# 14chanwa/remotesensingProject

Measured on AMD Instinct MI355X. Metric: Mpixel*disparity-hypotheses/s, higher is better.
Workload: dtype f32

## Files before the change

### remotesensingproject_amd/csrc/k2_reg.hpp

```cpp
#pragma once

#include "k2_scan.hpp"

namespace rslf {

#ifndef RSLF_REG_GB104
#define RSLF_REG_GB104 8
#endif
constexpr int gather_batch(int c) { return c == 1 ? 8 : 4; }
constexpr int kPadSlack = 16;

template <int SPAD, int C, bool BORDER, bool UNIFORM_D, bool PK, int GB = 0, class BestT = Best<C>, bool LANE_D = false>
__device__ __forceinline__ void scan_reg_body(const ScanArgs& a, int v, int u, int d0, int d1, BestT& best,
                                              float* __restrict__ otab, int dlane = 0, int dstep = 1)
{
    static_assert(!LANE_D || !UNIFORM_D, "hypotheses in the lanes: every lane has its own view offsets");
    constexpr int kGatherBatch = GB > 0 ? GB : (C == 1 && !PK && SPAD == 104 && RSLF_REG_GB104 == 13) ? 13 : gather_batch(C);
    static_assert(SPAD % kGatherBatch == 0 && (!PK || kGatherBatch % 2 == 0), "whole batches, whole pairs");
    static_assert(SPAD % 8 == 0, "slot counts are multiples of 8");
    const VolView& vol = a.vol;
    const float* epi = vol.row(v, 0);
    const float uf = (float)u;
    const int Um1 = vol.U - 1;
    const unsigned Um1_bits = __float_as_uint((float)Um1);
    const int S = vol.S;
    const int lane = threadIdx.x & 63;
    const long long o = (long long)v * vol.U + u;
    const float dmin = a.dmin_vu ? a.dmin_vu[o] : a.dmin;
    const float dmax = a.dmax_vu ? a.dmax_vu[o] : a.dmax;
    const float range = dmax - dmin;
    const float denom = (float)(a.dim_d - 1);
    const float kq = (C == 1) ? a.k.k1 : a.k.inv_h2;
    const float slope = a.k.slope;
    const int stride_s = (int)vol.stride_s;
    float centre[C];
#pragma unroll
    for (int c = 0; c < C; c++)
        centre[c] = epi[(long long)a.s_hat * vol.stride_s + u * C + c];

#pragma unroll 1
    for (int dk = d0; dk < d1; dk += (LANE_D ? dstep : 1)) {
        const int d = LANE_D ? min(dk + dlane, d1 - 1) : dk;
        const float Dd = hypothesis(dmin, range, denom, d);
        float R[PK ? 1 : C][PK ? 1 : SPAD];
        f2 R2[PK ? C : 1][PK ? SPAD / 2 : 1];
        int card = BORDER ? 0 : S;
        float Ss0 = (float)a.s_hat;
        asm volatile("" : "+v"(Ss0));
        int rowoff = 0;
        asm volatile("" : "+s"(rowoff));
        if (UNIFORM_D) {
#pragma unroll
            for (int s0 = 0; s0 < SPAD; s0 += 64) {
                const int s = s0 + lane;
                float off = (float)(a.s_hat - s) * Dd;
                off = off * slope;
                if (SPAD % 64 == 0 || s < SPAD)
                    otab[s] = off;
            }
            __builtin_amdgcn_wave_barrier();
        }
#pragma unroll
        for (int g = 0; g < SPAD / kGatherBatch; g++) {
            float tt[kGatherBatch], e0[C][kGatherBatch], e1[C][kGatherBatch];
            bool ok[kGatherBatch];
#pragma unroll
            for (int j = 0; j < kGatherBatch; j++) {
                const int s = g * kGatherBatch + j;
                tt[j] = 0.0f;
                ok[j] = false;
#pragma unroll
                for (int c = 0; c < C; c++) {
                    e0[c][j] = kSentinel;
                    e1[c][j] = 0.0f;
                }
                if (s < SPAD - kPadSlack || s < S) {
                    float x;
                    if (UNIFORM_D) {
                        x = otab[s];
                    } else {
                        x = (Ss0 - (float)s) * Dd;
                        x = x * slope;
                    }
                    x = x + uf;
                    tt[j] = lerp_weight(x);
                    int i0 = floor_to_int(x);
                    ok[j] = true;
                    if (BORDER) {
                        ok[j] = __float_as_uint(x) <= Um1_bits;
                        i0 = ok[j] ? i0 : 0;
                    }
                    const unsigned byteoff = (unsigned)(i0 * C + rowoff) << 2;
                    const float* p = (const float*)((const char*)epi + byteoff);
#pragma unroll
                    for (int c = 0; c < C; c++) {
                        e0[c][j] = p[c];
                        e1[c][j] = p[C + c];
                    }
                }
                rowoff += stride_s;
            }
#pragma unroll
            for (int j = 0; j < kGatherBatch; j++) {
                const int s = g * kGatherBatch + j;
                const float omt = 1.0f - tt[j];
#pragma unroll
                for (int c = 0; c < C; c++) {
                    const float m0 = omt * e0[c][j];
                    const float m1 = tt[j] * e1[c][j];
                    const float r = m0 + m1;
                    float val;
                    if (BORDER)
                        val = ok[j] ? r : kSentinel;
                    else
                        val = (s < SPAD - kPadSlack || s < S) ? r : kSentinel;
                    if constexpr (PK) {
                        if (s & 1)
                            R2[c][s >> 1].y = val;
                        else
                            R2[c][s >> 1].x = val;
                    } else {
                        R[c][s] = val;
                    }
                }
                if (BORDER)
                    card += ok[j] ? 1 : 0;
            }
            {
                const int b = g * kGatherBatch;
#pragma unroll
                for (int c = 0; c < C; c++) {
                    if constexpr (PK) {
                        asm volatile("" : "+v"(R2[c][b / 2]), "+v"(R2[c][b / 2 + 1]));
                        if (kGatherBatch == 8)
                            asm volatile("" : "+v"(R2[c][b / 2 + 2]), "+v"(R2[c][b / 2 + 3]));
                        static_assert(!PK || kGatherBatch == 4 || kGatherBatch == 8, "pair pinning is written for 4 and 8");
                    } else if (kGatherBatch != 4 && kGatherBatch != 8) {
#pragma unroll
                        for (int j = 0; j < kGatherBatch; j++)
                            asm volatile("" : "+v"(R[c][b + j]));
                    } else {
                        asm volatile("" : "+v"(R[c][b + 0]), "+v"(R[c][b + 1]), "+v"(R[c][b + 2]), "+v"(R[c][b + 3]));
                        if (kGatherBatch == 8)
                            asm volatile("" : "+v"(R[c][b + kGatherBatch - 4]), "+v"(R[c][b + kGatherBatch - 3]),
                                              "+v"(R[c][b + kGatherBatch - 2]), "+v"(R[c][b + kGatherBatch - 1]));
                    }
                }
                if (BORDER)
                    asm volatile("" : "+s"(rowoff), "+v"(Ss0), "+v"(card));
                else
                    asm volatile("" : "+s"(rowoff), "+v"(Ss0));
            }
        }

        float rbar[C];
#pragma unroll
        for (int c = 0; c < C; c++)
            rbar[c] = centre[c];
        float B = 0.0f;
#pragma unroll 1
        for (int it = 0; it < a.k.n_iter; it++) {
            float A[C];
#pragma unroll
            for (int c = 0; c < C; c++)
                A[c] = 0.0f;
            B = 0.0f;
            if constexpr (PK) {
                f2 rb2[C];
                const f2 kq2 = {kq, kq};
#pragma unroll
                for (int c = 0; c < C; c++)
                    rb2[c] = f2{rbar[c], rbar[c]};
                constexpr int kBlk = (C == 1) ? 8 : 4;
#pragma unroll
                for (int s0 = 0; s0 < SPAD; s0 += kBlk) {
                    if (!(s0 < SPAD - kPadSlack || s0 < S))
                        continue;
                    if constexpr (C == 1) {
                        f2 P[4], K[4];
                        const f2 r4[4] = {R2[0][s0 / 2], R2[0][s0 / 2 + 1], R2[0][s0 / 2 + 2], R2[0][s0 / 2 + 3]};
                        mean_shift_pk_octet(r4, rb2[0], kq2, P, K);
#pragma unroll
                        for (int j = 0; j < 4; j++) {
                            A[0] = A[0] + P[j].x;
                            B = B + K[j].x;
                            A[0] = A[0] + P[j].y;
                            B = B + K[j].y;
                        }
                    } else {
                        f2 Pa[3], Pb[3], Ka, Kb;
                        const f2 ra[3] = {R2[0][s0 / 2], R2[1][s0 / 2], R2[C - 1][s0 / 2]};
                        const f2 rb[3] = {R2[0][s0 / 2 + 1], R2[1][s0 / 2 + 1], R2[C - 1][s0 / 2 + 1]};
                        const f2 m[3] = {rb2[0], rb2[C > 1 ? 1 : 0], rb2[C - 1]};
                        mean_shift_pk_rgb_quad(ra, rb, m, kq2, Pa, Pb, Ka, Kb);
#pragma unroll
                        for (int c = 0; c < C; c++)
                            A[c] = A[c] + Pa[c].x;
                        B = B + Ka.x;
#pragma unroll
                        for (int c = 0; c < C; c++)
                            A[c] = A[c] + Pa[c].y;
                        B = B + Ka.y;
#pragma unroll
                        for (int c = 0; c < C; c++)
                            A[c] = A[c] + Pb[c].x;
                        B = B + Kb.x;
#pragma unroll
                        for (int c = 0; c < C; c++)
                            A[c] = A[c] + Pb[c].y;
                        B = B + Kb.y;
                    }
                }
            } else if (C == 1) {
#pragma unroll
                for (int s0 = 0; s0 < SPAD; s0 += 4) {
                    if (s0 + 4 <= SPAD - kPadSlack || s0 + 4 <= S) {
                        mean_shift_group4(R[0][s0], R[0][s0 + 1], R[0][s0 + 2], R[0][s0 + 3], rbar[0], kq, A[0], B);
                    } else {
#pragma unroll
                        for (int j = 0; j < 3; j++)
                            if (s0 + j < S)
                                mean_shift_group1(R[0][s0 + j], rbar[0], kq, A[0], B);
                    }
                }
            } else {
#pragma unroll
                for (int s = 0; s < SPAD; s++) {
                    if (!(s < SPAD - kPadSlack || s < S))
                        continue;
                    float q[C];
#pragma unroll
                    for (int c = 0; c < C; c++) {
                        const float delta = R[c][s] - rbar[c];
                        const float tq = kq * delta;
                        q[c] = tq * delta;
                    }
                    float qs = q[0];
                    if (C == 3) {
                        qs = q[0] + q[C - 1];
                        qs = qs + q[C > 1 ? 1 : 0];
                    }
                    const float K = kernel_weight(qs);
#pragma unroll
                    for (int c = 0; c < C; c++) {
                        const float pr = R[c][s] * K;
                        A[c] = A[c] + pr;
                    }
                    B = B + K;
                }
            }
#pragma unroll
            for (int c = 0; c < C; c++) {
                const float qd = (B != 0.0f) ? (A[c] / B) : 0.0f;
                rbar[c] = (qd > 0.0f) ? qd : 0.0f;
            }
        }
        const float cardf = (float)card;
        float sc = (card != 0) ? (B / cardf) : 0.0f;
        sc = (sc > 0.0f) ? sc : 0.0f;
        if (!LANE_D || dk + dlane < d1)
            best.offer(sc, d, Dd, rbar);
    }
}

constexpr int scan_reg_waves(int spad, int c)
{
    const int regs = ((c * spad + (c == 1 ? 64 : 96) + 7) / 8) * 8;
    const int w = 512 / regs;
    if (c == 1 && spad > 104 && spad <= 144) return 3;
    if (c == 1 && spad >= 80 && spad <= 88) return 4;
    if (c == 3 && spad >= 32 && spad <= 40) return 3;
    if (c == 1 && (spad == 48 || spad == 40)) return 5;
    if (c == 3 && spad == 24) return 4;
    if (c == 1 && spad == 16) return 7;
    return w > 8 ? 8 : (w < 1 ? 1 : w);
}

#ifndef RSLF_REG_BEST_LDS
#define RSLF_REG_BEST_LDS 1
#endif
constexpr bool scan_reg_best_in_lds(int spad, int c)
{
    if (!RSLF_REG_BEST_LDS)
        return false;
    if (c == 1)
        return spad == 16 || spad == 40 || spad == 48 || (spad >= 80 && spad <= 88) || (spad >= 104 && spad <= 144);
    return spad == 24 || spad == 40;
}

constexpr bool scan_reg_packed_math(int spad, int c) { return scan_reg_waves(spad, c) == 1; }

template <int SPAD, int C, class BestT>
__device__ __forceinline__ void scan_reg_rows(const ScanArgs& a, int v, int u, int d0, int d1, BestT& best, float* otab)
{
    constexpr bool PK = scan_reg_packed_math(SPAD, C);
    if (a.dmin_vu) {
        scan_reg_body<SPAD, C, true, false, PK, 0, BestT>(a, v, u, d0, d1, best, otab);
        return;
    }
    const float max_ds = (float)max(a.s_hat, a.vol.S - 1 - a.s_hat);
    const float range = a.dmax - a.dmin, denom = (float)(a.dim_d - 1);
    const float uf = (float)u, Um1 = (float)(a.vol.U - 1);
    auto interior = [&](int d) -> bool {
        const float reach = max_ds * fabsf(hypothesis(a.dmin, range, denom, d)) * fabsf(a.k.slope) + 2.0f;
        return __all((uf - reach >= 0.0f) && (uf + reach <= Um1));
    };
    int d = d0;
    while (d < d1) {
        const bool in = interior(d);
        int e = d + 1;
        while (e < d1 && interior(e) == in)
            e++;
        if (in)
            scan_reg_body<SPAD, C, false, true, PK, 0, BestT>(a, v, u, d, e, best, otab);
        else
            scan_reg_body<SPAD, C, true, true, PK, 0, BestT>(a, v, u, d, e, best, otab);
        d = e;
    }
}

template <int SPAD, int C>
__global__ __launch_bounds__(64 * kScanWaves) __attribute__((amdgpu_waves_per_eu(scan_reg_waves(SPAD, C), scan_reg_waves(SPAD, C))))
void k2_scan_reg(ScanArgs a)
{
    __shared__ float s_otab[kScanWaves][SPAD];
    float* otab = s_otab[__builtin_amdgcn_readfirstlane(threadIdx.x >> 6)];
    constexpr bool kEpiDyn = false;
    float* const epi_lds = nullptr;
    const int epi_stride = 0;
    if constexpr (scan_reg_best_in_lds(SPAD, C)) {
        __shared__ float s_best[kScanWaves][BestLds<C>::kFloats];
        BestLds<C> running(s_best[__builtin_amdgcn_readfirstlane(threadIdx.x >> 6)]);
        RSLF_SCAN_ROW_TILE((running.init(), scan_reg_rows<SPAD, C>(a, v, u, d0, d1, running, otab), running.load(best)))
    } else {
        RSLF_SCAN_ROW_TILE((scan_reg_rows<SPAD, C>(a, v, u, d0, d1, best, otab)))
    }
}

#ifndef RSLF_PACKED_LONG_GB
#define RSLF_PACKED_LONG_GB 4
#endif
constexpr bool packed_long_unit(int spad, int c) { return c == 1 && spad >= 80 && spad <= 128 && spad % RSLF_PACKED_LONG_GB == 0; }
constexpr int packed_waves(int spad, int c) { return packed_long_unit(spad, c) ? 2 : scan_reg_waves(spad + 24, c); }
constexpr int packed_gather_batch(int spad, int c) { return packed_long_unit(spad, c) ? spad / RSLF_PACKED_LONG_GB : 0; }

template <int SPAD, int C>
__global__ __launch_bounds__(64 * kScanWaves) __attribute__((amdgpu_waves_per_eu(packed_waves(SPAD, C), packed_waves(SPAD, C))))
void k2_scan_reg_packed(ScanArgs a)
{
    constexpr bool kEpiDyn = false;
    float* const epi_lds = nullptr;
    const int epi_stride = 0;
    RSLF_SCAN_PACKED_LOOP((scan_reg_body<SPAD, C, true, false, packed_waves(SPAD, C) == 1, packed_gather_batch(SPAD, C)>(a, v, u, d0, d1, best, nullptr)))
}

#ifndef RSLF_PX_ROWLIKE
#define RSLF_PX_ROWLIKE 1
#endif
constexpr int px_kernel_waves(int spad, int c) { return RSLF_PX_ROWLIKE ? scan_reg_waves(spad, c) : packed_waves(spad, c); }
template <int SPAD, int C>
__global__ __launch_bounds__(64 * kScanWaves) __attribute__((amdgpu_waves_per_eu(px_kernel_waves(SPAD, C), px_kernel_waves(SPAD, C))))
void k2_scan_reg_px(ScanArgs a)
{
    __shared__ double s_sum[kScanWaves];
    __shared__ float s_rec[kScanWaves][kPxRecFloats];
    const int n = *a.packed_n;
    const int lane = threadIdx.x & 63;
    const int wave = __builtin_amdgcn_readfirstlane(threadIdx.x >> 6);
    const int wpp = a.px_waves, ppw = kScanWaves / wpp;
    const int items = (n + ppw - 1) / ppw;
    const int sub = wave % wpp;
    const int dlane = sub * 64 + lane, dstep = 64 * wpp;
    for (int item = blockIdx.x; item < items; item += gridDim.x) {
        const int e = item * ppw + wave / wpp;
        const bool listed = e < n;
        const unsigned o = (unsigned)__builtin_amdgcn_readfirstlane(a.list[listed ? e : n - 1]);
        const int v = (int)(o / (unsigned)a.vol.U);
        const int u = (int)(o - (unsigned)v * (unsigned)a.vol.U);
        const bool have = listed && scan_px_owns(a, v);
        Best<C> best;
        best.init();
        const float dlo = a.dmin_vu ? a.dmin_vu[o] : a.dmin, dhi = a.dmax_vu ? a.dmax_vu[o] : a.dmax;
        const float reach = (float)max(a.s_hat, a.vol.S - 1 - a.s_hat) * fmaxf(fabsf(dlo), fabsf(dhi)) * fabsf(a.k.slope) + 2.0f;
        const bool interior = (float)u - reach >= 0.0f && (float)u + reach <= (float)(a.vol.U - 1);
        constexpr int kGB = RSLF_PX_ROWLIKE ? 0 : packed_gather_batch(SPAD, C);
        if (!have) {
        } else if (interior)
            scan_reg_body<SPAD, C, false, false, false, kGB, Best<C>, true>(a, v, u, 0, a.dim_d, best, nullptr, dlane, dstep);
        else
            scan_reg_body<SPAD, C, true, false, false, kGB, Best<C>, true>(a, v, u, 0, a.dim_d, best, nullptr, dlane, dstep);
        scan_px_finish<C>(a, o, have, best, wave, lane, wpp, s_rec, s_sum);
    }
}

}
```

### remotesensingproject_amd/csrc/k2_scan.hpp

```cpp
#pragma once

#include <type_traits>

#include "rslf_device.hpp"

namespace rslf {

constexpr int kScanWaves = 4;
#ifndef RSLF_XCD_ROW_INTERLEAVE
#define RSLF_XCD_ROW_INTERLEAVE 1
#endif

struct ScanArgs {
    VolView vol;
    const int* list;
    const int* count;
    const float* dmin_vu;
    const float* dmax_vu;
    float dmin, dmax;
    int dim_d, s_hat;
    ScanConsts k;
    float* Ce;
    uint8_t* Ce_mask;
    float* Cd;
// ... 85 lines not shown
            blk[0] = sc;
            reinterpret_cast<int*>(blk)[64] = dd;
            blk[128] = Dd;
#pragma unroll
            for (int c = 0; c < C; c++)
                blk[(3 + c) * 64] = rb[c];
        }
    }
    __device__ __forceinline__ void load(Best<C>& b) const
    {
        b.score = blk[0];
        b.d = reinterpret_cast<const int*>(blk)[64];
        b.D = blk[128];
#pragma unroll
        for (int c = 0; c < C; c++)
            b.rbar[c] = blk[(3 + c) * 64];
        b.sum = *sum_ptr();
    }
};

__device__ __forceinline__ bool scan_tile_span(const ScanArgs& a, int lb, int& v, int& e0, int& width, int& n)
{
    if (lb >= a.logical_blocks)
        return false;
    const int tile = lb / a.groups;
    const int vr = tile / a.tiles_per_row;
    const int j = tile - vr * a.tiles_per_row;
    v = vr + a.v0;
    n = a.count[v];
    if (j * a.tile_w >= n || n < a.row_min)
        return false;
    width = a.tile_w;
    if (a.tile_w == 63) {
        const int T = max(1, (n + 61) / 63);
        if (j >= T)
            return false;
        if (j == T - 1)
            width = n - 63 * j;
    }
    e0 = j * a.tile_w;
    return true;
}
__device__ __forceinline__ bool scan_tile(const ScanArgs& a, int lb, int& v, int& u, bool& active, int lane = threadIdx.x & 63)
{
    int e0, width, n;
    if (!scan_tile_span(a, lb, v, e0, width, n))
        return false;
    const int e = e0 + lane;
    active = lane < width && e < n;
    const int idx = active ? e : min(e0 + width, n) - 1;
    if (a.rowbase)
        u = a.list[a.rowbase[v] + idx] - v * a.vol.U;
    else
        u = a.list[(long long)v * a.vol.U + idx];
    return true;
}

__device__ __forceinline__ void scan_tile_packed(const ScanArgs& a, int item, int n, int& v, int& u, bool& active)
{
    const int lane = threadIdx.x & 63;
    const int e = (item / a.groups) * 64 + lane;
    active = e < n;
    const unsigned o = (unsigned)a.list[active ? e : n - 1];
    v = (int)(o / (unsigned)a.vol.U);
    u = (int)(o - (unsigned)v * (unsigned)a.vol.U);
}

__device__ __forceinline__ void scan_chunk(const ScanArgs& a, int group, int& d0, int& d1)
{
    const int wave = __builtin_amdgcn_readfirstlane(threadIdx.x >> 6);
    const int slices = kScanWaves * a.groups;
    const int chunk = (a.dim_d + slices - 1) / slices;
    d0 = min((group * kScanWaves + wave) * chunk, a.dim_d);
    d1 = min(d0 + chunk, a.dim_d);
}

__device__ __forceinline__ float hypothesis(float dmin, float range, float denom, int d)
{
    const float num = (float)d * range;
    const float quo = num / denom;
    return dmin + quo;
}

template <int C>
__device__ __forceinline__ void write_pixel(const ScanArgs& a, long long o, float best, int best_d, float best_D,
                                            const float (&best_rbar)[C], double sum)
{
    if ((double)best > (double)a.k.raw_thr) {
        a.depth[o] = best_D;
        const double mean = sum / (double)a.dim_d;
        a.Cd[o] = (float)((double)a.Ce[o] * fabs((double)best - mean));
#pragma unroll
        for (int c = 0; c < C; c++)
            a.rbar[o * C + c] = best_rbar[c];
        if (a.idx)
            a.idx[o] = best_d;
        if (a.score)
            a.score[o] = best;
    } else {
        a.Ce[o] = 0.0f;
        a.Ce_mask[o] = 0;
    }
}

constexpr int kPxRecFloats = 3 + 3;
__device__ __forceinline__ bool scan_px_owns(const ScanArgs& a, int v)
{
    return a.row_min == 0 || a.count[v] < a.row_min;
}

template <int C>
__device__ __forceinline__ void scan_px_finish(const ScanArgs& a, unsigned o, bool have, const Best<C>& best, int wave, int lane, int wpp,
                                               float (*rec)[kPxRecFloats], double* wsum)
{
    const int sub = wave % wpp;
    float bs = best.score;
    int bd = bs < 0.0f ? 0x7fffffff : best.d;
    double sum = best.sum;
#pragma unroll
    for (int m = 32; m >= 1; m >>= 1) {
        const float os = __shfl_xor(bs, m);
        const int od = __shfl_xor(bd, m);
        const bool take = os > bs || (os == bs && od < bd);
        bs = take ? os : bs;
        bd = take ? od : bd;
        sum += __shfl_xor(sum, m);
    }
    const int owner = __ffsll((unsigned long long)__ballot(best.score == bs && best.d == bd)) - 1;
    float bD = __shfl(best.D, owner);
    float br[C];
#pragma unroll
    for (int c = 0; c < C; c++)
        br[c] = __shfl(best.rbar[c], owner);
    if (wpp > 1) {
        if (lane == 0) {
            rec[wave][0] = bs;
            rec[wave][1] = __int_as_float(bd);
            rec[wave][2] = bD;
#pragma unroll
            for (int c = 0; c < C; c++)
                rec[wave][3 + c] = br[c];
            wsum[wave] = sum;
        }
        __syncthreads();
        if (sub == 0) {
            for (int w = wave + 1; w < wave + wpp; w++) {
                const float os = rec[w][0];
                const int od = __float_as_int(rec[w][1]);
                sum += wsum[w];
                if (os > bs || (os == bs && od < bd)) {
                    bs = os;
                    bd = od;
                    bD = rec[w][2];
#pragma unroll
                    for (int c = 0; c < C; c++)
                        br[c] = rec[w][3 + c];
                }
            }
        }
        __syncthreads();
    }
    if (have && sub == 0 && lane == 0)
        write_pixel<C>(a, (long long)o, bs, bd, bD, br, sum);
}

#if defined(__HIP_DEVICE_COMPILE__) && !defined(__gfx950__) && !defined(__gfx942__)
#error "k2_scan.hpp: the cross-workgroup record hand-off is written for gfx950 (gfx9 vmcnt / sc1 semantics); use agent-scope release/acquire fences on other targets"
#endif
__device__ __forceinline__ void store_coherent(unsigned* p, unsigned v)
{
    __hip_atomic_store(p, v, __ATOMIC_RELAXED, __HIP_MEMORY_SCOPE_AGENT);
}
__device__ __forceinline__ unsigned load_coherent(const unsigned* p)
{
    return __hip_atomic_load(p, __ATOMIC_RELAXED, __HIP_MEMORY_SCOPE_AGENT);
}

constexpr int kRecordWords = 8;

template <int C>
__device__ __forceinline__ void combine_tile(const ScanArgs& a, int tile, int v, int u, int lane);

template <int C>
struct EpilogueBlock {
    static constexpr int kDoubles = 64 + (3 + C) * 32;
    double* sum;
    float *score, *D, *rbar;
    int* d;
    __device__ __forceinline__ explicit EpilogueBlock(double* base)
        : sum(base), score(reinterpret_cast<float*>(base + 64)), D(score + 64), rbar(D + 64), d(reinterpret_cast<int*>(rbar + C * 64)) {}
};

template <int C, bool DYN = false>
__device__ __forceinline__ void scan_epilogue(const ScanArgs& a, int lb, int v, int u, bool active, const Best<C>& mine,
                                              float* wave_lds = nullptr, int wave_stride = 0, int lane = threadIdx.x & 63,
                                              int wave = threadIdx.x >> 6)
{
    __shared__ double s_static[DYN ? 1 : kScanWaves][DYN ? 1 : EpilogueBlock<C>::kDoubles];
    auto block_of = [&](int w) {
        return EpilogueBlock<C>(DYN ? reinterpret_cast<double*>(wave_lds + (long long)(w - wave) * wave_stride) : s_static[DYN ? 0 : w]);
    };
    {
        const EpilogueBlock<C> me = block_of(wave);
        me.score[lane] = mine.score;
        me.D[lane] = mine.D;
        me.d[lane] = mine.d;
        me.sum[lane] = mine.sum;
#pragma unroll
        for (int c = 0; c < C; c++)
            me.rbar[c * 64 + lane] = mine.rbar[c];
    }
    __syncthreads();
    if (wave != 0) {
        __syncthreads();
        return;
    }

    float best = mine.score, best_D = mine.D;
    int best_d = mine.d;
    float best_rbar[C];
#pragma unroll
    for (int c = 0; c < C; c++)
        best_rbar[c] = mine.rbar[c];
    double sum = mine.sum;
#pragma unroll
    for (int w = 1; w < kScanWaves; w++) {
        const EpilogueBlock<C> o = block_of(w);
        const float sc = o.score[lane];
        sum += o.sum[lane];
        if (sc > best || (sc == best && o.d[lane] < best_d)) {
            best = sc;
            best_d = o.d[lane];
            best_D = o.D[lane];
#pragma unroll
            for (int c = 0; c < C; c++)
                best_rbar[c] = o.rbar[c * 64 + lane];
        }
    }
    __syncthreads();
    if (a.groups > 1) {
        unsigned* w = reinterpret_cast<unsigned*>(a.partial) + ((long long)lb * kRecordWords * 64 + lane);
        static_assert(sizeof(Partial) == 4 * kRecordWords, "eight words per record");
        const unsigned long long sb = (unsigned long long)__double_as_longlong(sum);
        store_coherent(w + 0 * 64, __float_as_uint(best));
        store_coherent(w + 1 * 64, __float_as_uint(best_D));
        store_coherent(w + 2 * 64, (unsigned)best_d);
#pragma unroll
        for (int c = 0; c < C; c++)
            store_coherent(w + (3 + c) * 64, __float_as_uint(best_rbar[c]));
        store_coherent(w + 6 * 64, (unsigned)sb);
        store_coherent(w + 7 * 64, (unsigned)(sb >> 32));
        asm volatile("s_waitcnt vmcnt(0)" ::: "memory");
        const int tile = lb / a.groups;
        int drawn = 0;
        if (lane == 0)
            drawn = atomicAdd(&a.ticket[tile], 1);
        drawn = __builtin_amdgcn_readfirstlane(drawn);
        if (drawn != a.groups - 1)
            return;
        asm volatile("" ::: "memory");
        if (active)
            combine_tile<C>(a, tile, v, u, lane);
        if (lane == 0)
            a.ticket[tile] = 0;
        return;
    }
    if (active)
        write_pixel<C>(a, (long long)v * a.vol.U + u, best, best_d, best_D, best_rbar, sum);
}

template <int C>
__device__ __forceinline__ void combine_tile(const ScanArgs& a, int tile, int v, int u, int lane)
{
    const unsigned* pr = reinterpret_cast<const unsigned*>(a.partial) + ((long long)tile * a.groups * kRecordWords * 64 + lane);
    float best = -1.0f, best_D = 0.0f;
    int best_d = -1;
    float best_rbar[C];
#pragma unroll
    for (int c = 0; c < C; c++)
        best_rbar[c] = 0.0f;
    double sum = 0.0;
    constexpr int GB = 8, W = kRecordWords;
    for (int g0 = 0; g0 < a.groups; g0 += GB) {
        unsigned w[GB][W];
#pragma unroll
        for (int j = 0; j < GB; j++) {
            const unsigned* q = pr + (long long)min(g0 + j, a.groups - 1) * 64 * W;
#pragma unroll
            for (int k = 0; k < W; k++)
                if (k < 3 + C || k >= 6)
                    w[j][k] = load_coherent(q + k * 64);
        }
#pragma unroll
        for (int j = 0; j < GB; j++) {
            const int g = g0 + j;
            if (g >= a.groups)
                break;
            const float q_score = __uint_as_float(w[j][0]);
            const double q_sum = __longlong_as_double((long long)((unsigned long long)w[j][6] | ((unsigned long long)w[j][7] << 32)));
            sum = g == 0 ? q_sum : sum + q_sum;
            if (g == 0 || q_score > best) {
                best = q_score;
                best_D = __uint_as_float(w[j][1]);
                best_d = (int)w[j][2];
#pragma unroll
                for (int c = 0; c < C; c++)
                    best_rbar[c] = __uint_as_float(w[j][3 + c]);
            }
        }
    }
    write_pixel<C>(a, (long long)v * a.vol.U + u, best, best_d, best_D, best_rbar, sum);
}

template <int C>
__device__ __forceinline__ void scan_generic_body(const ScanArgs& a, int v, int u, int d0, int d1, Best<C>& best,
                                                  float* __restrict__ Kcol = nullptr, long long kstride = 0)
{
    const VolView& vol = a.vol;
    const float* epi = vol.row(v, 0);
    const float uf = (float)u;
    const int Um1 = vol.U - 1;
    const long long o = (long long)v * vol.U + u;
    const float dmin = a.dmin_vu ? a.dmin_vu[o] : a.dmin;
    const float dmax = a.dmax_vu ? a.dmax_vu[o] : a.dmax;
    const float range = dmax - dmin;
    const float denom = (float)(a.dim_d - 1);

    for (int d = d0; d < d1; d++) {
        const float Dd = hypothesis(dmin, range, denom, d);
        float rbar[C];
#pragma unroll
        for (int c = 0; c < C; c++) {
            rbar[c] = epi[(long long)a.s_hat * vol.stride_s + u * C + c];
            if (a.k.interp == 2 && u != 0)
                rbar[c] = NAN;
        }
        float B = 0.0f, card = 0.0f;
        for (int it = 0; it < a.k.n_iter; it++) {
            float A[C];
#pragma unroll
            for (int c = 0; c < C; c++)
                A[c] = 0.0f;
            B = 0.0f;
            card = 0.0f;
            for (int s = 0; s < vol.S; s++) {
                float x = (float)(a.s_hat - s) * Dd;
                x = x * a.k.slope;
                x = x + uf;
                const float fl = floorf(x);
                int i0 = (int)fl;
                int i1 = (int)ceilf(x);
                float t = x - fl;
                bool valid = !(i0 < 0 || i1 > Um1);
                if (a.k.interp != 0) {
                    int r;
                    if (a.k.interp == 2) {
                        r = __float_as_int(x);
                        valid = r > -1 && r < vol.U;
                    } else {
                        r = (int)roundf(x);
                        valid = fabsf(x) < 2.0e9f && r > -1 && r < vol.U;
                    }
                    i0 = i1 = r;
                    t = 0.0f;
                }
                const int j0 = min(max(i0, 0), Um1), j1 = min(max(i1, 0), Um1);
                const float* row = epi + (long long)s * vol.stride_s;
                const float omt = 1.0f - t;
                float K;
                float R0[C];
                if (C == 1) {
                    const float m0 = omt * row[j0];
                    const float m1 = t * row[j1];
                    float R = m0 + m1;
                    R = valid ? R : NAN;
                    R0[0] = (R > 0.0f) ? R : 0.0f;
                    const float delta = R - rbar[0];
                    const float q = (a.k.k1 * delta) * delta;
                    K = kernel_weight(q);
                } else {
                    float q[C];
#pragma unroll
                    for (int c = 0; c < C; c++) {
                        const float m0 = omt * row[j0 * C + c];
                        const float m1 = t * row[j1 * C + c];
                        float R = m0 + m1;
                        R = valid ? R : NAN;
                        R0[c] = (R > 0.0f) ? R : 0.0f;
                        const float delta = R - rbar[c];
                        q[c] = (a.k.inv_h2 * delta) * delta;
                    }
                    float qs = q[0] + q[C > 2 ? 2 : 0];
                    qs = qs + q[C > 1 ? 1 : 0];
                    K = kernel_weight(qs);
                }
#pragma unroll
                for (int c = 0; c < C; c++) {
                    const float pr = R0[c] * K;
                    A[c] = A[c] + pr;
                }
                B = B + K;
                card = card + (valid ? 1.0f : 0.0f);
                if (Kcol && it == a.k.n_iter - 1)
                    Kcol[(long long)s * kstride] = K;
            }
#pragma unroll
            for (int c = 0; c < C; c++) {
                const float q = (B != 0.0f) ? (A[c] / B) : 0.0f;
                rbar[c] = (q > 0.0f) ? q : 0.0f;
            }
        }
        float sc = (card != 0.0f) ? (B / card) : 0.0f;
        sc = (sc > 0.0f) ? sc : 0.0f;
        best.offer(sc, d, Dd, rbar);
    }
}

constexpr int kPackedItemTarget = 2048;
__device__ __forceinline__ int packed_groups(int groups, int tiles, int adapt)
{
    while (adapt && groups > 1 && tiles * groups > kPackedItemTarget)
        groups >>= 1;
    return groups;
}

#define RSLF_SCAN_PACKED_LOOP(PACKED_CALL) RSLF_SCAN_PACKED_LOOP_(scan_chunk, PACKED_CALL)
#define RSLF_SCAN_ROW_TILE(ROWS_CALL) RSLF_SCAN_ROW_TILE_(scan_chunk, ROWS_CALL)
#define RSLF_SCAN_PACKED_LOOP_(CHUNK, PACKED_CALL)                                      \
    {                                                                                   \
        const int n = *a.packed_n;                                                      \
        ScanArgs a_items = a;                                                           \
        a_items.groups = packed_groups(a.groups, (n + 63) >> 6, a.packed_adapt);        \
        {                                                                               \
            const ScanArgs& a = a_items;               \
            Best<C> best;                                                               \
            int v, u, d0, d1;                                                           \
            bool active;                                                                \
            const int items = ((n + 63) >> 6) * a.groups;                               \
            for (int item = blockIdx.x; item < items; item += gridDim.x) {              \
                scan_tile_packed(a, item, n, v, u, active);                             \
                CHUNK(a, item % a.groups, d0, d1);                                      \
                best.init();                                                            \
                PACKED_CALL;                                                            \
                scan_epilogue<C, kEpiDyn>(a, item, v, u, active, best, epi_lds, epi_stride); \
            }                                                                           \
        }                                                                               \
    }
#define RSLF_SCAN_ROW_TILE_(CHUNK, ROWS_CALL)                                           \
    {                                                                                   \
        Best<C> best;                                                                   \
        int v, u, d0, d1;                                                               \
        bool active;                                                                    \
        const int lb = RSLF_XCD_ROW_INTERLEAVE ? xcd_logical_block_rows(blockIdx.x, a.tiles_per_row * a.groups) \
                                               : xcd_logical_block(blockIdx.x, a.per_xcd); \
        if (!scan_tile(a, lb, v, u, active))                                            \
            return;                                                                     \
        CHUNK(a, lb % a.groups, d0, d1);                                                \
        best.init();                                                                    \
        ROWS_CALL;                                                                      \
        scan_epilogue<C, kEpiDyn>(a, lb, v, u, active, best, epi_lds, epi_stride);      \
    }
#define RSLF_SCAN_KERNEL_BODY_(CHUNK, ROWS_CALL, PACKED_CALL)                           \
    if (a.packed) {                                                                     \
        RSLF_SCAN_PACKED_LOOP_(CHUNK, PACKED_CALL)                                      \
        return;                                                                         \
    }                                                                                   \
    RSLF_SCAN_ROW_TILE_(CHUNK, ROWS_CALL)
#define RSLF_SCAN_KERNEL_BODY(ROWS_CALL, PACKED_CALL) RSLF_SCAN_KERNEL_BODY_(scan_chunk, ROWS_CALL, PACKED_CALL)

template <int C>
__global__ __launch_bounds__(64 * kScanWaves) void k2_scan_generic(ScanArgs a)
{
    constexpr bool kEpiDyn = false;
    float* const epi_lds = nullptr;
    const int epi_stride = 0;
    RSLF_SCAN_KERNEL_BODY((scan_generic_body<C>(a, v, u, d0, d1, best)), (scan_generic_body<C>(a, v, u, d0, d1, best)))
}

template <int C>
__global__ __launch_bounds__(256) void k2_kernel_column(ScanArgs a, const int32_t* __restrict__ idx_vu, float* __restrict__ K_vsu)
{
    const int v = blockIdx.y;
    const int u = blockIdx.x * blockDim.x + threadIdx.x;
    if (u >= a.vol.U)
        return;
    const int d = idx_vu[(long long)v * a.vol.U + u];
    if (d < 0)
        return;
    Best<C> best;
    best.init();
    scan_generic_body<C>(a, v, u, d, d + 1, best, K_vsu + (long long)v * a.vol.S * a.vol.U + u, (long long)a.vol.U);
}

int launch_scan_chip(const ScanArgs& a, dim3 grid, size_t lds_bytes, hipStream_t stream);

}
```

### remotesensingproject_amd/csrc/rslf_device.hpp

```cpp
#pragma once

#include <hip/hip_runtime.h>
#include <stdint.h>

namespace rslf {

constexpr int kWave = 64;
constexpr float kSentinel = 1.0e30f;

struct VolView {
    const float* base;
    int V, S, U, C;
    int pitch;
    long long stride_s;
    long long stride_v;
    __device__ __forceinline__ const float* row(int v, int s) const
    {
        return base + (long long)v * stride_v + (long long)s * stride_s;
    }
};

struct ScanConsts {
    float slope;
    float inv_h2;
// ... 101 lines not shown
        "v_pk_mul_f32 %[tb1], %[kq], %[db1]\n\t"
        "v_pk_mul_f32 %[tb2], %[kq], %[db2]\n\t"
        "v_pk_mul_f32 %[da0], %[da0], %[ta0]\n\t"
        "v_pk_mul_f32 %[da2], %[da2], %[ta2]\n\t"
        "v_pk_mul_f32 %[db0], %[db0], %[tb0]\n\t"
        "v_pk_mul_f32 %[db2], %[db2], %[tb2]\n\t"
        "v_pk_mul_f32 %[da1], %[da1], %[ta1]\n\t"
        "v_pk_mul_f32 %[db1], %[db1], %[tb1]\n\t"
        "v_pk_add_f32 %[da0], %[da0], %[da2]\n\t"
        "v_pk_add_f32 %[db0], %[db0], %[db2]\n\t"
        "v_pk_add_f32 %[da0], %[da0], %[da1]\n\t"
        "v_pk_add_f32 %[db0], %[db0], %[db1]\n\t"
        "v_pk_add_f32 %[ka], %[one], %[da0] neg_lo:[0,1] neg_hi:[0,1] clamp\n\t"
        "v_pk_add_f32 %[kb], %[one], %[db0] neg_lo:[0,1] neg_hi:[0,1] clamp\n\t"
        "v_pk_mul_f32 %[ta0], %[ra0], %[ka]\n\t"
        "v_pk_mul_f32 %[ta1], %[ra1], %[ka]\n\t"
        "v_pk_mul_f32 %[ta2], %[ra2], %[ka]\n\t"
        "v_pk_mul_f32 %[tb0], %[rb0], %[kb]\n\t"
        "v_pk_mul_f32 %[tb1], %[rb1], %[kb]\n\t"
        "v_pk_mul_f32 %[tb2], %[rb2], %[kb]"
        : [da0] "=&v"(da0), [da1] "=&v"(da1), [da2] "=&v"(da2), [db0] "=&v"(db0), [db1] "=&v"(db1), [db2] "=&v"(db2),
          [ta0] "=&v"(ta0), [ta1] "=&v"(ta1), [ta2] "=&v"(ta2), [tb0] "=&v"(tb0), [tb1] "=&v"(tb1), [tb2] "=&v"(tb2),
          [ka] "=&v"(Ka), [kb] "=&v"(Kb)
        : [ra0] "v"(ra[0]), [ra1] "v"(ra[1]), [ra2] "v"(ra[2]), [rb0] "v"(rb[0]), [rb1] "v"(rb[1]), [rb2] "v"(rb[2]),
          [m0] "v"(rbar[0]), [m1] "v"(rbar[1]), [m2] "v"(rbar[2]), [kq] "v"(kq), [one] "v"(one));
    Pa[0] = ta0;
    Pa[1] = ta1;
    Pa[2] = ta2;
    Pb[0] = tb0;
    Pb[1] = tb1;
    Pb[2] = tb2;
}

__device__ __forceinline__ void mean_shift_group4(float r0, float r1, float r2, float r3, float rbar, float k1,
                                                  float& A, float& B)
{
    float t0, t1, t2, t3, u0, u1, u2, u3;
    asm("v_sub_f32 %2, %10, %14\n\t"
        "v_sub_f32 %3, %11, %14\n\t"
        "v_sub_f32 %4, %12, %14\n\t"
        "v_sub_f32 %5, %13, %14\n\t"
        "v_mul_f32 %6, %15, %2\n\t"
        "v_mul_f32 %7, %15, %3\n\t"
        "v_mul_f32 %8, %15, %4\n\t"
        "v_mul_f32 %9, %15, %5\n\t"
        "v_mul_f32 %2, %2, %6\n\t"
        "v_mul_f32 %3, %3, %7\n\t"
        "v_mul_f32 %4, %4, %8\n\t"
        "v_mul_f32 %5, %5, %9\n\t"
        "v_sub_f32_e64 %2, 1.0, %2 clamp\n\t"
        "v_sub_f32_e64 %3, 1.0, %3 clamp\n\t"
        "v_sub_f32_e64 %4, 1.0, %4 clamp\n\t"
        "v_sub_f32_e64 %5, 1.0, %5 clamp\n\t"
        "v_mul_f32 %6, %10, %2\n\t"
        "v_mul_f32 %7, %11, %3\n\t"
        "v_mul_f32 %8, %12, %4\n\t"
        "v_mul_f32 %9, %13, %5\n\t"
        "v_add_f32 %0, %0, %6\n\t"
        "v_add_f32 %1, %1, %2\n\t"
        "v_add_f32 %0, %0, %7\n\t"
        "v_add_f32 %1, %1, %3\n\t"
        "v_add_f32 %0, %0, %8\n\t"
        "v_add_f32 %1, %1, %4\n\t"
        "v_add_f32 %0, %0, %9\n\t"
        "v_add_f32 %1, %1, %5"
        : "+v"(A), "+v"(B), "=&v"(t0), "=&v"(t1), "=&v"(t2), "=&v"(t3), "=&v"(u0), "=&v"(u1), "=&v"(u2), "=&v"(u3)
        : "v"(r0), "v"(r1), "v"(r2), "v"(r3), "v"(rbar), "s"(k1));
}

__device__ __forceinline__ void mean_shift_group1(float r0, float rbar, float k1, float& A, float& B)
{
    float t0, u0;
    asm("v_sub_f32 %2, %4, %5\n\t"
        "v_mul_f32 %3, %6, %2\n\t"
        "v_mul_f32 %2, %2, %3\n\t"
        "v_sub_f32_e64 %2, 1.0, %2 clamp\n\t"
        "v_mul_f32 %3, %4, %2\n\t"
        "v_add_f32 %0, %0, %3\n\t"
        "v_add_f32 %1, %1, %2"
        : "+v"(A), "+v"(B), "=&v"(t0), "=&v"(u0)
        : "v"(r0), "v"(rbar), "s"(k1));
}

__device__ __forceinline__ int reflect101(int p, int len)
{
    if (len == 1)
        return 0;
    while (p < 0 || p >= len)
        p = (p < 0) ? -p : 2 * len - 2 - p;
    return p;
}

__device__ __forceinline__ int xcd_logical_block(int b, int per_xcd)
{
    return (b & 7) * per_xcd + (b >> 3);
}

__device__ __forceinline__ int xcd_logical_block_rows(int b, int row_blocks)
{
    const int slot = b >> 3;
    const int k = slot / row_blocks;
    return ((b & 7) + 8 * k) * row_blocks + (slot - k * row_blocks);
}

}
```

Before: 8029.

## Skip rbar accumulation in final mean-shift pass; recompute winner rbar at write-out

For scalar one-channel register-scan variants, the last mean-shift iteration per hypothesis now accumulates only the kernel weight sum B (the score), dropping the A accumulation and the rbar divide. The rbar of the winning hypothesis is then recomputed once per pixel in the epilogue by re-gathering the view samples and running that final pass. This removes per-hypothesis ALU work in the hot loop, at the cost of an extra gather and pass per written pixel plus template plumbing through the epilogue and combine paths.

```diff
diff --git a/remotesensingproject_amd/csrc/k2_reg.hpp b/remotesensingproject_amd/csrc/k2_reg.hpp
--- a/remotesensingproject_amd/csrc/k2_reg.hpp
+++ b/remotesensingproject_amd/csrc/k2_reg.hpp
@@ -10,7 +10,106 @@
 constexpr int gather_batch(int c) { return c == 1 ? 8 : 4; }
 constexpr int kPadSlack = 16;
 
-template <int SPAD, int C, bool BORDER, bool UNIFORM_D, bool PK, int GB = 0, class BestT = Best<C>, bool LANE_D = false>
+template <int SPAD, int C, bool PK, bool KONLY>
+__device__ __forceinline__ void mean_shift_pass(const float (&R)[PK ? 1 : C][PK ? 1 : SPAD], const f2 (&R2)[PK ? C : 1][PK ? SPAD / 2 : 1],
+                                                int S, float kq, const float (&rbar)[C], float (&A)[C], float& B)
+{
+    static_assert(!KONLY || (C == 1 && !PK), "the K-only pass is written for the scalar one-channel blocks");
+    if constexpr (PK) {
+        f2 rb2[C];
+        const f2 kq2 = {kq, kq};
+#pragma unroll
+        for (int c = 0; c < C; c++)
+            rb2[c] = f2{rbar[c], rbar[c]};
+        constexpr int kBlk = (C == 1) ? 8 : 4;
+#pragma unroll
+        for (int s0 = 0; s0 < SPAD; s0 += kBlk) {
+            if (!(s0 < SPAD - kPadSlack || s0 < S))
+                continue;
+            if constexpr (C == 1) {
+                f2 P[4], K[4];
+                const f2 r4[4] = {R2[0][s0 / 2], R2[0][s0 / 2 + 1], R2[0][s0 / 2 + 2], R2[0][s0 / 2 + 3]};
+                mean_shift_pk_octet(r4, rb2[0], kq2, P, K);
+#pragma unroll
+                for (int j = 0; j < 4; j++) {
+                    A[0] = A[0] + P[j].x;
+                    B = B + K[j].x;
+                    A[0] = A[0] + P[j].y;
+                    B = B + K[j].y;
+                }
+            } else {
+                f2 Pa[3], Pb[3], Ka, Kb;
+                const f2 ra[3] = {R2[0][s0 / 2], R2[1][s0 / 2], R2[C - 1][s0 / 2]};
+                const f2 rb[3] = {R2[0][s0 / 2 + 1], R2[1][s0 / 2 + 1], R2[C - 1][s0 / 2 + 1]};
+                const f2 m[3] = {rb2[0], rb2[C > 1 ? 1 : 0], rb2[C - 1]};
+                mean_shift_pk_rgb_quad(ra, rb, m, kq2, Pa, Pb, Ka, Kb);
+#pragma unroll
+                for (int c = 0; c < C; c++)
+                    A[c] = A[c] + Pa[c].x;
+                B = B + Ka.x;
+#pragma unroll
+                for (int c = 0; c < C; c++)
+                    A[c] = A[c] + Pa[c].y;
+                B = B + Ka.y;
+#pragma unroll
+                for (int c = 0; c < C; c++)
+                    A[c] = A[c] + Pb[c].x;
+                B = B + Kb.x;
+#pragma unroll
+                for (int c = 0; c < C; c++)
+                    A[c] = A[c] + Pb[c].y;
+                B = B + Kb.y;
+            }
+        }
+    } else if (C == 1) {
+#pragma unroll
+        for (int s0 = 0; s0 < SPAD; s0 += 4) {
+            if (s0 + 4 <= SPAD - kPadSlack || s0 + 4 <= S) {
+                if constexpr (KONLY)
+                    mean_shift_group4_k(R[0][s0], R[0][s0 + 1], R[0][s0 + 2], R[0][s0 + 3], rbar[0], kq, B);
+                else
+                    mean_shift_group4(R[0][s0], R[0][s0 + 1], R[0][s0 + 2], R[0][s0 + 3], rbar[0], kq, A[0], B);
+            } else {
+#pragma unroll
+                for (int j = 0; j < 3; j++)
+                    if (s0 + j < S) {
+                        if constexpr (KONLY)
+                            mean_shift_group1_k(R[0][s0 + j], rbar[0], kq, B);
+                        else
+                            mean_shift_group1(R[0][s0 + j], rbar[0], kq, A[0], B);
+                    }
+            }
+        }
+    } else {
+#pragma unroll
+        for (int s = 0; s < SPAD; s++) {
+            if (!(s < SPAD - kPadSlack || s < S))
+                continue;
+            float q[C];
+#pragma unroll
+            for (int c = 0; c < C; c++) {
+                const float delta = R[c][s] - rbar[c];
+                const float tq = kq * delta;
+                q[c] = tq * delta;
+            }
+            float qs = q[0];
+            if (C == 3) {
+                qs = q[0] + q[C - 1];
+                qs = qs + q[C > 1 ? 1 : 0];
+            }
+            const float K = kernel_weight(qs);
+#pragma unroll
+            for (int c = 0; c < C; c++) {
+                const float pr = R[c][s] * K;
+                A[c] = A[c] + pr;
+            }
+            B = B + K;
+        }
+    }
+}
+
+template <int SPAD, int C, bool BORDER, bool UNIFORM_D, bool PK, int GB = 0, class BestT = Best<C>, bool LANE_D = false,
+          bool TRIM = false>
 __device__ __forceinline__ void scan_reg_body(const ScanArgs& a, int v, int u, int d0, int d1, BestT& best,
                                               float* __restrict__ otab, int dlane = 0, int dstep = 1)
 {
@@ -165,90 +264,13 @@
             for (int c = 0; c < C; c++)
                 A[c] = 0.0f;
             B = 0.0f;
-            if constexpr (PK) {
-                f2 rb2[C];
-                const f2 kq2 = {kq, kq};
-#pragma unroll
-                for (int c = 0; c < C; c++)
-                    rb2[c] = f2{rbar[c], rbar[c]};
-                constexpr int kBlk = (C == 1) ? 8 : 4;
-#pragma unroll
-                for (int s0 = 0; s0 < SPAD; s0 += kBlk) {
-                    if (!(s0 < SPAD - kPadSlack || s0 < S))
-                        continue;
-                    if constexpr (C == 1) {
-                        f2 P[4], K[4];
-                        const f2 r4[4] = {R2[0][s0 / 2], R2[0][s0 / 2 + 1], R2[0][s0 / 2 + 2], R2[0][s0 / 2 + 3]};
-                        mean_shift_pk_octet(r4, rb2[0], kq2, P, K);
-#pragma unroll
-                        for (int j = 0; j < 4; j++) {
-                            A[0] = A[0] + P[j].x;
-                            B = B + K[j].x;
-                            A[0] = A[0] + P[j].y;
-                            B = B + K[j].y;
-                        }
-                    } else {
-                        f2 Pa[3], Pb[3], Ka, Kb;
-                        const f2 ra[3] = {R2[0][s0 / 2], R2[1][s0 / 2], R2[C - 1][s0 / 2]};
-                        const f2 rb[3] = {R2[0][s0 / 2 + 1], R2[1][s0 / 2 + 1], R2[C - 1][s0 / 2 + 1]};
-                        const f2 m[3] = {rb2[0], rb2[C > 1 ? 1 : 0], rb2[C - 1]};
-                        mean_shift_pk_rgb_quad(ra, rb, m, kq2, Pa, Pb, Ka, Kb);
-#pragma unroll
-                        for (int c = 0; c < C; c++)
-                            A[c] = A[c] + Pa[c].x;
-                        B = B + Ka.x;
-#pragma unroll
-                        for (int c = 0; c < C; c++)
-                            A[c] = A[c] + Pa[c].y;
-                        B = B + Ka.y;
-#pragma unroll
-                        for (int c = 0; c < C; c++)
-                            A[c] = A[c] + Pb[c].x;
-                        B = B + Kb.x;
-#pragma unroll
-                        for (int c = 0; c < C; c++)
-                            A[c] = A[c] + Pb[c].y;
-                        B = B + Kb.y;
-                    }
-                }
-            } else if (C == 1) {
-#pragma unroll
-                for (int s0 = 0; s0 < SPAD; s0 += 4) {
-                    if (s0 + 4 <= SPAD - kPadSlack || s0 + 4 <= S) {
-                        mean_shift_group4(R[0][s0], R[0][s0 + 1], R[0][s0 + 2], R[0][s0 + 3], rbar[0], kq, A[0], B);
-                    } else {
-#pragma unroll
-                        for (int j = 0; j < 3; j++)
-                            if (s0 + j < S)
-                                mean_shift_group1(R[0][s0 + j], rbar[0], kq, A[0], B);
-                    }
-                }
-            } else {
-#pragma unroll
-                for (int s = 0; s < SPAD; s++) {
-                    if (!(s < SPAD - kPadSlack || s < S))
-                        continue;
-                    float q[C];
-#pragma unroll
-                    for (int c = 0; c < C; c++) {
-                        const float delta = R[c][s] - rbar[c];
-                        const float tq = kq * delta;
-                        q[c] = tq * delta;
-                    }
-                    float qs = q[0];
-                    if (C == 3) {
-                        qs = q[0] + q[C - 1];
-                        qs = qs + q[C > 1 ? 1 : 0];
-                    }
-                    const float K = kernel_weight(qs);
-#pragma unroll
-                    for (int c = 0; c < C; c++) {
-                        const float pr = R[c][s] * K;
-                        A[c] = A[c] + pr;
-                    }
-                    B = B + K;
-                }
-            }
+            if constexpr (TRIM) {
+                if (it == a.k.n_iter - 1) {
+                    mean_shift_pass<SPAD, C, PK, true>(R, R2, S, kq, rbar, A, B);
+                    break;
+                }
+            }
+            mean_shift_pass<SPAD, C, PK, false>(R, R2, S, kq, rbar, A, B);
 #pragma unroll
             for (int c = 0; c < C; c++) {
                 const float qd = (B != 0.0f) ? (A[c] / B) : 0.0f;
@@ -262,6 +284,82 @@
             best.offer(sc, d, Dd, rbar);
     }
 }
+
+template <int C>
+struct LastPassRbar {
+    __device__ __forceinline__ void operator()(const ScanArgs& a, long long o, float Dd, float (&rbar)[C]) const
+    {
+        if (a.k.n_iter == 0)
+            return;
+        const VolView& vol = a.vol;
+        const int v = (int)(o / vol.U);
+        const int u = (int)(o - (long long)v * vol.U);
+        const float* epi = vol.row(v, 0);
+        const float uf = (float)u;
+        const unsigned Um1_bits = __float_as_uint((float)(vol.U - 1));
+        const float kq = (C == 1) ? a.k.k1 : a.k.inv_h2;
+        const float Ss0 = (float)a.s_hat;
+        const int S = vol.S;
+        float A[C];
+#pragma unroll
+        for (int c = 0; c < C; c++)
+            A[c] = 0.0f;
+        float B = 0.0f;
+        constexpr int kBatch = 8;
+#pragma unroll 1
+        for (int s0 = 0; s0 < S; s0 += kBatch) {
+            float R[C][kBatch];
+#pragma unroll
+            for (int j = 0; j < kBatch; j++) {
+                const int s = min(s0 + j, S - 1);
+                float x = (Ss0 - (float)s) * Dd;
+                x = x * a.k.slope;
+                x = x + uf;
+                const float t = lerp_weight(x);
+                const bool ok = __float_as_uint(x) <= Um1_bits;
+                const int i0 = ok ? floor_to_int(x) : 0;
+                const float* p = epi + (long long)s * vol.stride_s + i0 * C;
+                const float omt = 1.0f - t;
+#pragma unroll
+                for (int c = 0; c < C; c++) {
+                    const float m0 = omt * p[c];
+                    const float m1 = t * p[C + c];
+                    const float r = m0 + m1;
+                    R[c][j] = ok ? r : kSentinel;
+                }
+            }
+#pragma unroll
+            for (int j = 0; j < kBatch; j++) {
+                if (s0 + j >= S)
+                    break;
+                float q[C];
+#pragma unroll
+                for (int c = 0; c < C; c++) {
+                    const float delta = R[c][j] - rbar[c];
+                    const float tq = kq * delta;
+                    q[c] = tq * delta;
+                }
+                float qs = q[0];
+                if (C == 3) {
+                    qs = q[0] + q[C - 1];
+                    qs = qs + q[C > 1 ? 1 : 0];
+                }
+                const float K = kernel_weight(qs);
+#pragma unroll
+                for (int c = 0; c < C; c++) {
+                    const float pr = R[c][j] * K;
+                    A[c] = A[c] + pr;
+                }
+                B = B + K;
+            }
+        }
+#pragma unroll
+        for (int c = 0; c < C; c++) {
+            const float qd = (B != 0.0f) ? (A[c] / B) : 0.0f;
+            rbar[c] = (qd > 0.0f) ? qd : 0.0f;
+        }
+    }
+};
 
 constexpr int scan_reg_waves(int spad, int c)
 {
@@ -290,12 +388,19 @@
 
 constexpr bool scan_reg_packed_math(int spad, int c) { return scan_reg_waves(spad, c) == 1; }
 
+constexpr bool scan_reg_trim(int spad, int c)
+{
+    return c == 1 && !scan_reg_packed_math(spad, c) && spad != 48 && !(spad >= 80 && spad <= 88) && !(spad > 112 && spad <= 144);
+}
+template <int SPAD, int C>
+using ScanRegRbarFix = std::conditional_t<scan_reg_trim(SPAD, C), LastPassRbar<C>, NoRbarFix>;
+
 template <int SPAD, int C, class BestT>
 __device__ __forceinline__ void scan_reg_rows(const ScanArgs& a, int v, int u, int d0, int d1, BestT& best, float* otab)
 {
     constexpr bool PK = scan_reg_packed_math(SPAD, C);
     if (a.dmin_vu) {
-        scan_reg_body<SPAD, C, true, false, PK, 0, BestT>(a, v, u, d0, d1, best, otab);
+        scan_reg_body<SPAD, C, true, false, PK, 0, BestT, false, scan_reg_trim(SPAD, C)>(a, v, u, d0, d1, best, otab);
         return;
     }
     const float max_ds = (float)max(a.s_hat, a.vol.S - 1 - a.s_hat);
@@ -312,9 +417,9 @@
         while (e < d1 && interior(e) == in)
             e++;
         if (in)
-            scan_reg_body<SPAD, C, false, true, PK, 0, BestT>(a, v, u, d, e, best, otab);
+            scan_reg_body<SPAD, C, false, true, PK, 0, BestT, false, scan_reg_trim(SPAD, C)>(a, v, u, d, e, best, otab);
         else
-            scan_reg_body<SPAD, C, true, true, PK, 0, BestT>(a, v, u, d, e, best, otab);
+            scan_reg_body<SPAD, C, true, true, PK, 0, BestT, false, scan_reg_trim(SPAD, C)>(a, v, u, d, e, best, otab);
         d = e;
     }
 }
@@ -328,12 +433,13 @@
     constexpr bool kEpiDyn = false;
     float* const epi_lds = nullptr;
     const int epi_stride = 0;
+    using Fix = ScanRegRbarFix<SPAD, C>;
     if constexpr (scan_reg_best_in_lds(SPAD, C)) {
         __shared__ float s_best[kScanWaves][BestLds<C>::kFloats];
         BestLds<C> running(s_best[__builtin_amdgcn_readfirstlane(threadIdx.x >> 6)]);
-        RSLF_SCAN_ROW_TILE((running.init(), scan_reg_rows<SPAD, C>(a, v, u, d0, d1, running, otab), running.load(best)))
+        RSLF_SCAN_ROW_TILE_FIX((running.init(), scan_reg_rows<SPAD, C>(a, v, u, d0, d1, running, otab), running.load(best)), Fix{})
     } else {
-        RSLF_SCAN_ROW_TILE((scan_reg_rows<SPAD, C>(a, v, u, d0, d1, best, otab)))
+        RSLF_SCAN_ROW_TILE_FIX((scan_reg_rows<SPAD, C>(a, v, u, d0, d1, best, otab)), Fix{})
     }
 }
 
diff --git a/remotesensingproject_amd/csrc/k2_scan.hpp b/remotesensingproject_amd/csrc/k2_scan.hpp
--- a/remotesensingproject_amd/csrc/k2_scan.hpp
+++ b/remotesensingproject_amd/csrc/k2_scan.hpp
@@ -191,17 +191,27 @@
     return dmin + quo;
 }
 
-template <int C>
+struct NoRbarFix {
+    template <int C>
+    __device__ __forceinline__ void operator()(const ScanArgs&, long long, float, float (&)[C]) const {}
+};
+
+template <int C, class Fix = NoRbarFix>
 __device__ __forceinline__ void write_pixel(const ScanArgs& a, long long o, float best, int best_d, float best_D,
-                                            const float (&best_rbar)[C], double sum)
+                                            const float (&best_rbar)[C], double sum, const Fix& fix = Fix{})
 {
     if ((double)best > (double)a.k.raw_thr) {
         a.depth[o] = best_D;
         const double mean = sum / (double)a.dim_d;
         a.Cd[o] = (float)((double)a.Ce[o] * fabs((double)best - mean));
+        float rb[C];
 #pragma unroll
         for (int c = 0; c < C; c++)
-            a.rbar[o * C + c] = best_rbar[c];
+            rb[c] = best_rbar[c];
+        fix(a, o, best_D, rb);
+#pragma unroll
+        for (int c = 0; c < C; c++)
+            a.rbar[o * C + c] = rb[c];
         if (a.idx)
             a.idx[o] = best_d;
         if (a.score)
@@ -287,8 +297,8 @@
 
 constexpr int kRecordWords = 8;
 
-template <int C>
-__device__ __forceinline__ void combine_tile(const ScanArgs& a, int tile, int v, int u, int lane);
+template <int C, class Fix>
+__device__ __forceinline__ void combine_tile(const ScanArgs& a, int tile, int v, int u, int lane, const Fix& fix);
 
 template <int C>
 struct EpilogueBlock {
@@ -300,10 +310,10 @@
         : sum(base), score(reinterpret_cast<float*>(base + 64)), D(score + 64), rbar(D + 64), d(reinterpret_cast<int*>(rbar + C * 64)) {}
 };
 
-template <int C, bool DYN = false>
+template <int C, bool DYN = false, class Fix = NoRbarFix>
 __device__ __forceinline__ void scan_epilogue(const ScanArgs& a, int lb, int v, int u, bool active, const Best<C>& mine,
                                               float* wave_lds = nullptr, int wave_stride = 0, int lane = threadIdx.x & 63,
-                                              int wave = threadIdx.x >> 6)
+                                              int wave = threadIdx.x >> 6, const Fix& fix = Fix{})
 {
     __shared__ double s_static[DYN ? 1 : kScanWaves][DYN ? 1 : EpilogueBlock<C>::kDoubles];
     auto block_of = [&](int w) {
@@ -369,17 +379,17 @@
             return;
         asm volatile("" ::: "memory");
         if (active)
-            combine_tile<C>(a, tile, v, u, lane);
+            combine_tile<C>(a, tile, v, u, lane, fix);
         if (lane == 0)
             a.ticket[tile] = 0;
         return;
     }
     if (active)
-        write_pixel<C>(a, (long long)v * a.vol.U + u, best, best_d, best_D, best_rbar, sum);
-}
-
-template <int C>
-__device__ __forceinline__ void combine_tile(const ScanArgs& a, int tile, int v, int u, int lane)
+        write_pixel<C>(a, (long long)v * a.vol.U + u, best, best_d, best_D, best_rbar, sum, fix);
+}
+
+template <int C, class Fix>
+__device__ __forceinline__ void combine_tile(const ScanArgs& a, int tile, int v, int u, int lane, const Fix& fix)
 {
     const unsigned* pr = reinterpret_cast<const unsigned*>(a.partial) + ((long long)tile * a.groups * kRecordWords * 64 + lane);
     float best = -1.0f, best_D = 0.0f;
@@ -418,7 +428,7 @@
             }
         }
     }
-    write_pixel<C>(a, (long long)v * a.vol.U + u, best, best_d, best_D, best_rbar, sum);
+    write_pixel<C>(a, (long long)v * a.vol.U + u, best, best_d, best_D, best_rbar, sum, fix);
 }
 
 template <int C>
@@ -534,7 +544,8 @@
 }
 
 #define RSLF_SCAN_PACKED_LOOP(PACKED_CALL) RSLF_SCAN_PACKED_LOOP_(scan_chunk, PACKED_CALL)
-#define RSLF_SCAN_ROW_TILE(ROWS_CALL) RSLF_SCAN_ROW_TILE_(scan_chunk, ROWS_CALL)
+#define RSLF_SCAN_ROW_TILE(ROWS_CALL) RSLF_SCAN_ROW_TILE_(scan_chunk, ROWS_CALL, NoRbarFix{})
+#define RSLF_SCAN_ROW_TILE_FIX(ROWS_CALL, FIX) RSLF_SCAN_ROW_TILE_(scan_chunk, ROWS_CALL, FIX)
 #define RSLF_SCAN_PACKED_LOOP_(CHUNK, PACKED_CALL)                                      \
     {                                                                                   \
         const int n = *a.packed_n;                                                      \
@@ -555,7 +566,7 @@
             }                                                                           \
         }                                                                               \
     }
-#define RSLF_SCAN_ROW_TILE_(CHUNK, ROWS_CALL)                                           \
+#define RSLF_SCAN_ROW_TILE_(CHUNK, ROWS_CALL, FIX)                                      \
     {                                                                                   \
         Best<C> best;                                                                   \
         int v, u, d0, d1;                                                               \
@@ -567,14 +578,15 @@
         CHUNK(a, lb % a.groups, d0, d1);                                                \
         best.init();                                                                    \
         ROWS_CALL;                                                                      \
-        scan_epilogue<C, kEpiDyn>(a, lb, v, u, active, best, epi_lds, epi_stride);      \
+        scan_epilogue<C, kEpiDyn>(a, lb, v, u, active, best, epi_lds, epi_stride,       \
+                                  threadIdx.x & 63, threadIdx.x >> 6, FIX);             \
     }
 #define RSLF_SCAN_KERNEL_BODY_(CHUNK, ROWS_CALL, PACKED_CALL)                           \
     if (a.packed) {                                                                     \
         RSLF_SCAN_PACKED_LOOP_(CHUNK, PACKED_CALL)                                      \
         return;                                                                         \
     }                                                                                   \
-    RSLF_SCAN_ROW_TILE_(CHUNK, ROWS_CALL)
+    RSLF_SCAN_ROW_TILE_(CHUNK, ROWS_CALL, NoRbarFix{})
 #define RSLF_SCAN_KERNEL_BODY(ROWS_CALL, PACKED_CALL) RSLF_SCAN_KERNEL_BODY_(scan_chunk, ROWS_CALL, PACKED_CALL)
 
 template <int C>
diff --git a/remotesensingproject_amd/csrc/rslf_device.hpp b/remotesensingproject_amd/csrc/rslf_device.hpp
--- a/remotesensingproject_amd/csrc/rslf_device.hpp
+++ b/remotesensingproject_amd/csrc/rslf_device.hpp
@@ -207,6 +207,45 @@
         : "v"(r0), "v"(rbar), "s"(k1));
 }
 
+__device__ __forceinline__ void mean_shift_group4_k(float r0, float r1, float r2, float r3, float rbar, float k1, float& B)
+{
+    float t0, t1, t2, t3, u0, u1, u2, u3;
+    asm("v_sub_f32 %1, %9, %13\n\t"
+        "v_sub_f32 %2, %10, %13\n\t"
+        "v_sub_f32 %3, %11, %13\n\t"
+        "v_sub_f32 %4, %12, %13\n\t"
+        "v_mul_f32 %5, %14, %1\n\t"
+        "v_mul_f32 %6, %14, %2\n\t"
+        "v_mul_f32 %7, %14, %3\n\t"
+        "v_mul_f32 %8, %14, %4\n\t"
+        "v_mul_f32 %1, %1, %5\n\t"
+        "v_mul_f32 %2, %2, %6\n\t"
+        "v_mul_f32 %3, %3, %7\n\t"
+        "v_mul_f32 %4, %4, %8\n\t"
+        "v_sub_f32_e64 %1, 1.0, %1 clamp\n\t"
+        "v_sub_f32_e64 %2, 1.0, %2 clamp\n\t"
+        "v_add_f32 %0, %0, %1\n\t"
+        "v_sub_f32_e64 %3, 1.0, %3 clamp\n\t"
+        "v_add_f32 %0, %0, %2\n\t"
+        "v_sub_f32_e64 %4, 1.0, %4 clamp\n\t"
+        "v_add_f32 %0, %0, %3\n\t"
+        "v_add_f32 %0, %0, %4"
+        : "+v"(B), "=&v"(t0), "=&v"(t1), "=&v"(t2), "=&v"(t3), "=&v"(u0), "=&v"(u1), "=&v"(u2), "=&v"(u3)
+        : "v"(r0), "v"(r1), "v"(r2), "v"(r3), "v"(rbar), "s"(k1));
+}
+
+__device__ __forceinline__ void mean_shift_group1_k(float r0, float rbar, float k1, float& B)
+{
+    float t0, u0;
+    asm("v_sub_f32 %1, %3, %4\n\t"
+        "v_mul_f32 %2, %5, %1\n\t"
+        "v_mul_f32 %1, %1, %2\n\t"
+        "v_sub_f32_e64 %1, 1.0, %1 clamp\n\t"
+        "v_add_f32 %0, %0, %1"
+        : "+v"(B), "=&v"(t0), "=&v"(u0)
+        : "v"(r0), "v"(rbar), "s"(k1));
+}
+
 __device__ __forceinline__ int reflect101(int p, int len)
 {
     if (len == 1)
```

Result: faster. 8186, median of 6 (+2.0%).
